# Visual-Behavior/detr-tensorflow

Measured on AMD Instinct MI355X. Metric: images/sec training step, DETR-R50 800x1333 bs=8/GPU, higher is better.
Workload: dtype bf16

## Files before the change

detr-tensorflow_amd/detr_tf/_hip.py:

```python
import ctypes
import os
from ctypes import POINTER, Structure, byref, c_float, c_int32, c_int64, c_size_t, c_void_p

import torch

_HERE = os.path.dirname(os.path.abspath(__file__))
LIB_PATH = os.environ.get("DETR_HIP_LIB") or os.path.join(os.path.dirname(_HERE), "lib", "libdetr_hip.so")

f32p = c_void_p


class ReduceDesc(Structure):
    _fields_ = [("ws", c_void_p), ("splits", c_int32), ("part_stride", c_int64), ("rows", c_int32), ("cols", c_int32),
                ("C", c_void_p), ("ldc", c_int64), ("alpha", c_float), ("scale", c_void_p),
                ("rs_ws", c_void_p), ("rs_out", c_void_p), ("rs_alpha", c_float),
                ("ts_bm", c_int32), ("ts_bn", c_int32), ("ts_tiles_n", c_int32)]


class GemmDesc(Structure):
    _fields_ = [("M", c_int32), ("N", c_int32), ("K", c_int32),
                ("A", c_void_p), ("lda", c_int64), ("a_kcontig", c_int32),
                ("B", c_void_p), ("ldb", c_int64), ("b_kcontig", c_int32),
                ("C", c_void_p), ("ldc", c_int64),
                ("batch", c_int32), ("batch_inner", c_int32),
# ... 179 lines not shown

class SetLossDesc(Structure):
    _fields_ = [("levels", c_int32), ("B", c_int32), ("Q", c_int32), ("C", c_int32), ("R", c_int32),
                ("logits", c_void_p), ("sL_l", c_int64), ("sL_b", c_int64), ("sL_q", c_int64),
                ("boxes", c_void_p), ("sB_l", c_int64), ("sB_b", c_int64), ("sB_q", c_int64),
                ("t_bbox", c_void_p), ("t_class", c_void_p),
                ("background_class", c_int32)]


_SIGNATURES = {
    "detr_hip_abi_version": [],
    "detr_hip_reload_tuning": [],
    "detr_hip_struct_layout": [c_int32, POINTER(c_int32), c_int32],
    "detr_hip_memset_zero": [c_void_p, c_size_t, c_void_p],
    "detr_hip_gemm_f32": [POINTER(GemmDesc), c_void_p],
    "detr_hip_gemm_group_f32": [POINTER(GemmDesc), c_int32, c_void_p],
    "detr_hip_gemm_family": [POINTER(GemmDesc)],
    "detr_hip_gemm_ring_plan": [c_int32, c_int32, c_int32, POINTER(c_int32)],
    "detr_hip_splitk_reduce_many": [POINTER(ReduceDesc), c_int32, c_void_p],
    "detr_hip_conv3x3_f32": [POINTER(Conv3x3Desc), c_int32, c_void_p],
    "detr_hip_maxpool3x3s2_fwd_bf16": [c_void_p, c_void_p, c_void_p, c_int32, c_int32, c_int32, c_int32, c_int32, c_int32, c_void_p],
    "detr_hip_maxpool3x3s2_bwd_bf16": [c_void_p, c_void_p, c_void_p, c_void_p, c_int32, c_int32, c_int32, c_int32, c_int32, c_int32,
                                       c_void_p],
    "detr_hip_cvt_bf16": [f32p, c_void_p, c_int64, c_void_p],
    "detr_hip_scale_cols_bf16": [f32p, f32p, c_void_p, c_int64, c_int32, c_void_p],
    "detr_hip_scale_cols_bf16_group": [c_void_p, c_int32, c_void_p],
    "detr_hip_stem_conv7x7_f32": [POINTER(StemDesc), c_int32, c_void_p],
    "detr_hip_maxpool3x3s2_fwd_f32": [f32p, f32p, c_void_p, c_int32, c_int32, c_int32, c_int32, c_int32, c_int32, c_void_p],
    "detr_hip_maxpool3x3s2_bwd_f32": [f32p, c_void_p, f32p, f32p, c_int32, c_int32, c_int32, c_int32, c_int32, c_int32, c_void_p],
    "detr_hip_subsample2_fwd_f32": [f32p, f32p, c_int32, c_int32, c_int32, c_int32, c_int32, c_int32, c_void_p],
    "detr_hip_subsample2_bwd_f32": [f32p, f32p, c_int32, c_int32, c_int32, c_int32, c_int32, c_int32, c_void_p],
    "detr_hip_layernorm_fwd": [POINTER(LayerNormDesc), c_void_p],
    "detr_hip_layernorm_bwd": [POINTER(LayerNormDesc), c_void_p],
    "detr_hip_attention_fwd": [POINTER(AttnDesc), c_void_p],
    "detr_hip_attention_bwd": [POINTER(AttnDesc), c_void_p],
    "detr_hip_attention_dropmask": [POINTER(AttnDesc), c_void_p],
    "detr_hip_attention_dropmask_many": [POINTER(AttnDesc), c_int32, c_void_p],
    "detr_hip_attention_fwd_masked": [POINTER(AttnDesc), c_void_p, c_void_p],
    "detr_hip_attention_bwd_masked": [POINTER(AttnDesc), c_void_p, c_void_p],
    "detr_hip_attention_weights": [POINTER(AttnDesc), c_void_p, c_void_p, c_int64, c_void_p],
    "detr_hip_padding_mask_prepare": [c_void_p, c_int32, c_int32, c_int32, c_int32, c_int32, f32p, f32p, c_void_p, f32p, c_void_p, c_void_p],
    "detr_hip_input_stage_padded": [c_void_p, c_void_p, c_void_p, c_int32, c_int32, c_int32, f32p, c_void_p, f32p, c_void_p, c_void_p],
    "detr_hip_dropout_f32": [f32p, f32p, c_int64, c_float, ctypes.c_uint32, c_void_p, c_void_p],
    "detr_hip_multi_copy": [c_void_p, c_int32, c_int32, c_void_p],
    "detr_hip_colsum_scaled": [c_void_p, c_int32, c_int64, c_int32, c_int64, c_void_p, c_void_p, c_void_p],
    "detr_hip_fma_vec_group": [c_void_p, c_int32, c_void_p],
    "detr_hip_set_u32x8": [c_void_p] + [ctypes.c_uint32] * 8 + [c_void_p],
    "detr_hip_colsum_f32": [f32p, f32p, c_int64, c_int32, c_int64, c_float, c_void_p],
    "detr_hip_colsum_det_f32": [f32p, f32p, c_int64, c_int32, c_int64, c_float, f32p, c_int64, c_void_p],
    "detr_hip_conv1x1_bwd_fused_bf16": [c_void_p, c_int64, c_void_p, c_int64, c_void_p, c_int64, c_void_p, c_int64, c_int32, f32p, c_int64, f32p, c_float,
                                        c_int64, c_int32, c_int32, f32p, c_int64, c_void_p],
    "detr_hip_add_bcast_f32": [f32p, f32p, f32p, c_int64, c_int64, c_void_p],
    "detr_hip_add_f32": [f32p, f32p, f32p, c_int64, c_void_p],
    "detr_hip_sigmoid_bwd_f32": [f32p, f32p, f32p, c_int64, c_void_p],
    "detr_hip_relu_mask_f32": [f32p, f32p, f32p, c_int64, c_void_p],
    "detr_hip_scale_cols_f32": [f32p, f32p, f32p, c_int64, c_int32, c_void_p],
    "detr_hip_scale_cols_t_f32": [f32p, f32p, f32p, c_int32, c_int32, c_void_p],
    "detr_hip_bn_fold_f32": [f32p, f32p, f32p, f32p, f32p, f32p, c_int32, c_float, c_void_p],
    "detr_hip_postprocess": [POINTER(PostprocessDesc), c_void_p],
    "detr_hip_map_match": [POINTER(MapMatchDesc), c_void_p],
    "detr_hip_input_stage": [POINTER(InputDesc), c_void_p],
    "detr_hip_pad_labels": [c_void_p, c_void_p, c_void_p, c_int32, c_int32, c_void_p, c_void_p, c_void_p],
    "detr_hip_augment": [c_void_p, c_int64, c_void_p, f32p, c_int32, c_int32, c_int32, f32p, c_void_p, f32p, c_void_p],
    "detr_hip_augment_padded": [c_void_p, c_int64, c_void_p, c_int32, c_int32, c_int32, f32p, c_void_p, f32p, c_void_p, c_void_p],
    "detr_hip_match_cost_f32": [POINTER(SetLossDesc), f32p, c_void_p],
    "detr_hip_assign_f32": [f32p, c_int32, c_int32, c_int32, f32p, c_int32, c_int32, c_void_p, c_void_p, c_void_p, c_void_p],
    "detr_hip_set_loss_sums_f32": [POINTER(SetLossDesc), c_void_p, f32p, c_void_p],
    "detr_hip_set_loss_finalize_f32": [f32p, c_int32, f32p, f32p, c_void_p],
    "detr_hip_set_loss_grad_f32": [POINTER(SetLossDesc), c_void_p, f32p, c_float, f32p, f32p, c_void_p],
    "detr_hip_sumsq_segments_f32": [f32p, c_void_p, c_void_p, c_void_p, c_int32, c_int32, f32p, c_void_p],
    "detr_hip_clip_adam_f32": [f32p, f32p, f32p, f32p, c_void_p, c_void_p, c_void_p, c_void_p, f32p, f32p, c_int32, c_int32, c_void_p],
    "detr_hip_axpy_f32": [f32p, f32p, c_float, c_int64, c_void_p],
    "detr_hip_set_floats8_f32": [f32p] + [c_float] * 8 + [c_void_p],
    "detr_hip_set_floats16_f32": [f32p, POINTER(c_float * 16), c_void_p],
    "detr_hip_global_clip_scale_f32": [f32p, c_void_p, c_void_p, f32p, c_int32, f32p, c_void_p],
    "detr_hip_adamw_f32": [f32p, f32p, f32p, f32p, c_void_p, c_void_p, c_void_p, c_void_p, f32p, f32p, f32p, c_int32, c_int32, c_void_p],
    "detr_hip_conv3x3_dilated": [POINTER(Conv3x3DDesc), c_int32, c_void_p],
    "detr_hip_detect": [POINTER(DetectDesc), c_void_p],
    "detr_hip_tile_merge": [POINTER(TileMergeDesc), c_void_p],
    "detr_hip_coco_match": [POINTER(CocoMatchDesc), c_void_p],
    "detr_hip_overlay": [POINTER(OverlayDesc), c_void_p],
    "detr_hip_track": [POINTER(TrackDesc), c_void_p],
    "detr_hip_track_embed": [POINTER(TrackEmbedDesc), c_void_p],
}
_SIGNATURES_I64 = {
    "detr_hip_attention_dropmask_words": [c_int32, c_int32, c_int32, c_int32],
    "detr_hip_attention_keymask_words": [c_int32, c_int32],
    "detr_hip_colsum_det_scratch_floats": [c_int64, c_int32],
    "detr_hip_conv1x1_bwd_fused_workspace_floats": [c_int64],
    "detr_hip_workspace_bytes_gemm": [POINTER(GemmDesc)],
    "detr_hip_workspace_bytes_conv3x3": [POINTER(Conv3x3Desc), c_int32],
    "detr_hip_workspace_bytes_stem": [POINTER(StemDesc), c_int32],
    "detr_hip_workspace_bytes_layernorm": [POINTER(LayerNormDesc)],
    "detr_hip_workspace_bytes_conv3x3_dilated": [POINTER(Conv3x3DDesc), c_int32],
    "detr_hip_workspace_bytes_overlay": [POINTER(OverlayDesc)],
    "detr_hip_track_state_bytes": [c_int32],
    "detr_hip_track_embed_state_bytes": [c_int32, c_int32],
    "detr_hip_workspace_bytes_track_embed": [POINTER(TrackEmbedDesc)],
}
EXPORTED_SYMBOLS = sorted(list(_SIGNATURES) + list(_SIGNATURES_I64) + ["detr_hip_last_error"])
ABI_VERSION = 9
LAYOUT_STRUCTS = {0: ReduceDesc, 1: GemmDesc, 2: Conv3x3Desc, 3: StemDesc, 4: LayerNormDesc, 5: AttnDesc, 6: SetLossDesc, 7: InputDesc,
                  8: PostprocessDesc, 9: MapMatchDesc, 100: DetectDesc, 200: TileMergeDesc, 300: OverlayDesc}
LAYOUT_STRUCTS_APPENDED = {400: TrackDesc}
LAYOUT_STRUCTS_APPENDED_500 = {500: TrackEmbedDesc}

_lib = None


class KernelProfiler:

    def __init__(self, prealloc=0, f32=False):
        self.f32 = f32
        self.records = []
        self._pool = []
        for _ in range(prealloc):
            ev = torch.cuda.Event(enable_timing=True)
            ev.record()
            self._pool.append(ev)

    def _event(self):
        return self._pool.pop() if self._pool else torch.cuda.Event(enable_timing=True)

    def begin(self):
        ev = self._event()
        ev.record()
        return ev

    def end(self, family, flops, ev0, sig=None, nbytes=0.0):
        ev1 = self._event()
        ev1.record()
        self.records.append((family, flops, ev0, ev1, sig, nbytes))

    def by_shape(self, top=40):
        torch.cuda.synchronize()
        agg = {}
        for fam, flops, e0, e1, sig, _nb in self.records:
            d = agg.setdefault((fam, sig), [0, 0.0, 0.0])
            d[0] += 1
            d[1] += e0.elapsed_time(e1)
            d[2] += flops
        rows = sorted(agg.items(), key=lambda kv: -kv[1][1])[:top]
        return [{"family": k[0], "shape": k[1], "launches": v[0], "ms": round(v[1], 3),
                 "tflops": round(v[2] / (v[1] * 1e-3) / 1e12, 2) if v[1] > 0 else 0.0} for k, v in rows]

    def summary(self):
        torch.cuda.synchronize()
        out = {}
        for fam, flops, e0, e1, _sig, nb in self.records:
            d = out.setdefault(fam, {"launches": 0, "ms": 0.0, "flops": 0.0, "bytes": 0.0, "mixed_s": 0.0})
            d["launches"] += 1
            d["ms"] += e0.elapsed_time(e1)
            d["flops"] += flops
            d["bytes"] += nb
            d["mixed_s"] += max(flops / (157.3e12 if fam.startswith("gemm_f32") or self.f32 else 2.5e15), nb / 8.0e12)
        return out


PROFILER = None
DEFER = None
DEFER_WS = None
_defer_top = 0
_defer_outs = set()
COMPUTE_BF16 = 0
WORKSPACE = None

# ... 290 lines not shown
    if COMPUTE_BF16 == 1 and ((N >= 128 and K >= 16384) or (M >= 512 and N >= 512 and K >= 4096) or
                         (K >= 4096 and ((M >= 256 and N >= 2048) or (M >= 2048 and N >= 256)))):
        tiles = -(-M // 128) * -(-N // 128)
        ktiles = -(-K // 32)
        return int(max(1, min(max(1, SPLIT_TARGET_128 // tiles), max_split, ktiles // 8 if ktiles >= 16 else 1)))
    if COMPUTE_BF16 == 2 and X3_SPLIT_TARGET > 0 and N >= 128 and K >= 256 and M >= 128:
        t128 = -(-M // 128) * -(-N // 128)
        ktiles = -(-K // 32)
        cap = ktiles // 8 if ktiles >= 64 else max(1, ktiles // 4)
        s128 = int(max(1, min(X3_SPLIT_TARGET // t128, max_split, cap)))
        if t128 * s128 >= 192:
            return s128
    tiles = -(-M // 64) * -(-N // 64)
    want = max(1, SPLIT_TARGET_64 // max(tiles, 1))
    ktiles = -(-K // (32 if COMPUTE_BF16 == 1 else 16))
    cap = ktiles // 8 if ktiles >= 64 else ktiles // 4
    return int(max(1, min(want, max_split, cap)))


def linear_fwd_call(x2d, w_out_in, bias, out2d, *, alpha=1.0, residual=None, act=0, dropout_p=0.0, dropout_seed=0,
                    dropout_step=None, ln=None):
    M, K = x2d.shape
    N = w_out_in.shape[0]
    return ((M, N, K, x2d, x2d.stride(0), 1, w_out_in, w_out_in.stride(0), 1, out2d, out2d.stride(0)),
            dict(alpha=alpha, bias=bias, residual=residual, ldr=(residual.stride(0) if residual is not None else 0), act=act,
                 dropout_p=dropout_p, dropout_seed=dropout_seed, dropout_step=dropout_step, **({"ln": ln} if ln is not None else {})))


def linear_dgrad_call(dy2d, w_out_in, dx2d, *, alpha=1.0, residual=None, mask=None):
    M, N = dy2d.shape
    K = w_out_in.shape[1]
    return ((M, K, N, dy2d, dy2d.stride(0), 1, w_out_in, w_out_in.stride(0), 0, dx2d, dx2d.stride(0)),
            dict(alpha=alpha, residual=residual, ldr=(residual.stride(0) if residual is not None else 0),
                 mask=mask, ldmask=(mask.stride(0) if mask is not None else 0)))


def linear_wgrad_call(dy2d, x2d, dw_out_in, *, alpha=1.0, bias_grad=None):
    M, N = dy2d.shape
    K = x2d.shape[1]
    sk = pick_split_k(N, K, M)
    args = (N, K, M, dy2d, dy2d.stride(0), 0, x2d, x2d.stride(0), 0, dw_out_in, dw_out_in.stride(0))
    if sk == 1:
        return args, dict(alpha=alpha, residual=dw_out_in, ldr=dw_out_in.stride(0), rowsum_a=bias_grad, rowsum_alpha=alpha)
    return args, dict(alpha=alpha, split_k=sk, rowsum_a=bias_grad, rowsum_alpha=alpha)


def linear_fwd(*a, **kw):
    args, kwargs = linear_fwd_call(*a, **kw)
    gemm(*args, **kwargs)


def linear_dgrad(*a, **kw):
    args, kwargs = linear_dgrad_call(*a, **kw)
    gemm(*args, **kwargs)


def linear_wgrad(*a, **kw):
    args, kwargs = linear_wgrad_call(*a, **kw)
    gemm(*args, **kwargs)


def conv1x1_bwd_fused_scratch_floats(M):
    return int(load().detr_hip_conv1x1_bwd_fused_workspace_floats(int(M)))


def conv1x1_bwd_fused(dy, a, w, da, dw, scratch, *, scale=None, use_mask=True, alpha=1.0):
    M = dy.shape[0]
    for t, shape, dt in ((dy, (M, 256), torch.bfloat16), (a, (M, 64), torch.bfloat16), (w, (64, 256), torch.bfloat16), (da, (M, 64), torch.bfloat16),
                         (dw, (64, 256), torch.float32)):
        if tuple(t.shape) != shape or t.dtype != dt or t.stride(1) != 1:
            raise ValueError(f"conv1x1_bwd_fused: operand of shape {tuple(t.shape)} / {t.dtype} / strides {t.stride()}, expected {shape} {dt}, unit column stride")
    if scratch.dtype != torch.float32 or (scale is not None and (scale.dtype != torch.float32 or scale.numel() != 256)):
        raise ValueError("conv1x1_bwd_fused: scratch / scale must be fp32 (scale: 256 entries)")
    ev0 = PROFILER.begin() if PROFILER is not None else None
    _check(load().detr_hip_conv1x1_bwd_fused_bf16(dy.data_ptr(), dy.stride(0), a.data_ptr(), a.stride(0), w.data_ptr(), w.stride(0), da.data_ptr(),
                                                  da.stride(0), 1 if use_mask else 0, dw.data_ptr(), dw.stride(0), ptr(scale), c_float(alpha), M,
                                                  a.shape[1], dy.shape[1], scratch.data_ptr(), scratch.numel(), _stream()),
           "detr_hip_conv1x1_bwd_fused_bf16")
    if ev0 is not None:
        PROFILER.end("conv1x1_bwd_fused", 4.0 * M * a.shape[1] * dy.shape[1], ev0, f"M{M} {a.shape[1]}->{dy.shape[1]}",
                     float(2 * M * (dy.shape[1] + 2 * a.shape[1])))


def conv3x3(mode, x, w, y, N, Hi, Wi, Ci, Ho, Wo, Co, stride, *, pad=1, alpha=1.0, scale=None, bias=None,
            residual=None, mask=None, act=0, split=0, compute=None, maskbits_out=None, dilation=1):
    if dilation not in (1, 2):
        raise ValueError(f"conv3x3: dilation {dilation} unsupported (1 or 2)")
    dil = dilation == 2
    d = Conv3x3DDesc() if dil else Conv3x3Desc()
    if dil:
        d.dilation = 2
    fn, ws_fn = ("detr_hip_conv3x3_dilated", "detr_hip_workspace_bytes_conv3x3_dilated") if dil else \
        ("detr_hip_conv3x3_f32", "detr_hip_workspace_bytes_conv3x3")
    d.N, d.Hi, d.Wi, d.Ci, d.Ho, d.Wo, d.Co, d.stride, d.pad = N, Hi, Wi, Ci, Ho, Wo, Co, stride, pad
    d.x, d.w, d.y = x.data_ptr(), w.data_ptr(), y.data_ptr()
    is16 = lambda t: 1 if (t is not None and t.dtype == torch.bfloat16) else 0
    d.w_dtype, d.x_dtype, d.y_dtype, d.r_dtype, d.m_dtype = is16(w), is16(x), is16(y), is16(residual), is16(mask)
    if mask is not None and mask.dtype == torch.uint8:
        d.m_dtype = 2
    d.maskbits_out = ptr(maskbits_out)
    d.alpha = alpha
    d.scale, d.bias, d.residual, d.mask = ptr(scale), ptr(bias), ptr(residual), ptr(mask)
    d.act, d.split = act, split
    d.compute = COMPUTE_BF16 if compute is None else int(compute)
    if mode == 2 and WORKSPACE is not None:
        need_workspace(_ws_query(ws_fn, ("convd" if dil else "conv", N, Hi, Wi, Ci, Ho, Wo, Co, stride, pad, split, d.compute, d.x_dtype),
                                 byref(d), mode))
    d.workspace, d.workspace_bytes = (WORKSPACE.data_ptr(), WORKSPACE.numel() * 4) if WORKSPACE is not None else (None, 0)
    ev0 = PROFILER.begin() if PROFILER is not None else None
    _check(getattr(load(), fn)(byref(d), mode, _stream()), fn)
    if ev0 is not None:
        rows = N * (Hi * Wi if mode == 1 else Ho * Wo)
        PROFILER.end(("conv3x3_fwd", "conv3x3_dgrad", "conv3x3_wgrad")[mode], 2.0 * (N * Ho * Wo) * 9 * Ci * Co, ev0,
                     f"N{N} {Hi}x{Wi}x{Ci}->{Ho}x{Wo}x{Co} s{stride}" + (" d2" if dil else ""),
                     float(x.element_size() * (N * Hi * Wi * Ci if mode != 1 else N * Ho * Wo * Co)
                           + (w.element_size() * 9 * Ci * Co if mode != 2 else w.element_size() * N * Ho * Wo * Co)
                           + y.element_size() * (N * Ho * Wo * Co if mode == 0 else (N * Hi * Wi * Ci if mode == 1 else 9 * Ci * Co))
                           + ((rows * (Ci if mode == 1 else Co) // 8 if mask.dtype == torch.uint8 else mask.element_size() * rows * (Ci if mode == 1 else Co))
                              if mask is not None else 0) + (rows * Co // 8 if maskbits_out is not None else 0)
                           + (residual.element_size() * rows * (Ci if mode == 1 else Co) if residual is not None else 0)))


def stem_conv(mode, img, w, y, N, H, W, Ho, Wo, *, alpha=1.0, scale=None, bias=None, act=0, split=0, compute=None):
    d = StemDesc()
    d.N, d.H, d.W, d.Ho, d.Wo = N, H, W, Ho, Wo
    d.img, d.w, d.y = img.data_ptr(), w.data_ptr(), y.data_ptr()
    d.alpha = alpha
    d.scale, d.bias = ptr(scale), ptr(bias)
    d.act, d.split = act, split
    d.w_dtype = 1 if (mode == 2 and w.dtype == torch.bfloat16) else 0
    d.y_dtype = 1 if (mode == 0 and y.dtype == torch.bfloat16) else 0
    d.compute = COMPUTE_BF16 if compute is None else int(compute)
    if mode == 2 and WORKSPACE is not None:
        need_workspace(_ws_query("detr_hip_workspace_bytes_stem", ("stem", N, H, W, Ho, Wo, split, d.compute, d.w_dtype), byref(d), mode))
    d.workspace, d.workspace_bytes = (WORKSPACE.data_ptr(), WORKSPACE.numel() * 4) if WORKSPACE is not None else (None, 0)
    ev0 = PROFILER.begin() if PROFILER is not None else None
    _check(load().detr_hip_stem_conv7x7_f32(byref(d), mode, _stream()), "detr_hip_stem_conv7x7_f32")
    if ev0 is not None:
        M = N * Ho * Wo
        PROFILER.end("stem_conv7x7", 2.0 * M * 64 * 147, ev0, f"stem7x7 mode{mode} M{M}",
                     float(4 * N * H * W * 3 + (y if mode == 0 else w).element_size() * M * 64 + 4 * 147 * 64))


def call(name, *args):
    _check(getattr(load(), name)(*args, _stream()), name)


def zero_(t):
    call("detr_hip_memset_zero", t.data_ptr(), t.numel() * t.element_size())
    return t


def attention_dropmask_words(B, H, T, S):
    return int(load().detr_hip_attention_dropmask_words(B, H, T, S))


def attention_keymask_words(B, S):
    return int(load().detr_hip_attention_keymask_words(B, S))


def keymask_words_from_valid(valid):
    import numpy as np
    valid = np.asarray(valid, dtype=bool)
    B, S = valid.shape
    nw = (S + 31) // 32
    bits = np.zeros((B, nw * 32), dtype=np.uint64)
# ... 180 lines not shown
```

detr-tensorflow_amd/detr_tf/engine.py:

```python
import math
import os
from ctypes import byref, c_float

import numpy as np
import torch

from . import _hip as hip
from .params import ParamStore, RESNET50_BLOCKS, block_names, bn_conv_pairs, stem_names

D = 256
HEADS = 8
HD = 32
FF = 2048
BN_EPS = 1e-5
KERAS_BN_EPS = 1.001e-5
LN_EPS = 1e-5
DEFER_REDUCE = os.environ.get("DETR_HIP_DEFER_REDUCE", "1") != "0"
WGRAD_STREAM = os.environ.get("DETR_HIP_WGRAD_STREAM", "1") != "0"
BWD_FUSED = os.environ.get("DETR_HIP_BWD_FUSED", "1") != "0"
DROPMASK_AHEAD = int(os.environ.get("DETR_HIP_DROPMASK_AHEAD", "2") or 0)
QK_ALPHA = float(HD) ** -0.5 * 1.4426950408889634


def mix32(x):
    x &= 0xFFFFFFFF
    x ^= x >> 16
    x = (x * 0x7FEB352D) & 0xFFFFFFFF
    x ^= x >> 15
    x = (x * 0x846CA68B) & 0xFFFFFFFF
    x ^= x >> 16
    return x


def step_seed(base_seed, step_no, rank=0):
    return mix32(mix32((base_seed + 0x9E3779B9 * step_no) & 0xFFFFFFFF) ^ ((rank * 0x85EBCA6B) & 0xFFFFFFFF))


def position_embedding_sine_host(H, W, num_pos_features=128, temperature=10000.0, eps=1e-6):
    y = (np.arange(1, H + 1, dtype=np.float32) / np.float32(H + eps) * np.float32(2 * math.pi)).astype(np.float32)
    x = (np.arange(1, W + 1, dtype=np.float32) / np.float32(W + eps) * np.float32(2 * math.pi)).astype(np.float32)
    k = np.arange(num_pos_features, dtype=np.float32)
    dim_t = np.power(np.float32(temperature), (2 * np.floor(k / 2) / np.float32(num_pos_features)).astype(np.float32)).astype(np.float32)
    py = (y[:, None] / dim_t[None, :]).astype(np.float32)
    px = (x[:, None] / dim_t[None, :]).astype(np.float32)
    ey = np.empty_like(py)
    ex = np.empty_like(px)
    ey[:, 0::2], ey[:, 1::2] = np.sin(py[:, 0::2]), np.cos(py[:, 1::2])
    ex[:, 0::2], ex[:, 1::2] = np.sin(px[:, 0::2]), np.cos(px[:, 1::2])
    pos = np.concatenate([np.broadcast_to(ey[:, None, :], (H, W, num_pos_features)),
                          np.broadcast_to(ex[None, :, :], (H, W, num_pos_features))], axis=2)
    return np.ascontiguousarray(pos.reshape(H * W, 2 * num_pos_features), dtype=np.float32)


def position_embedding_sine_table(n_max, num_pos_features=128, temperature=10000.0, eps=1e-6):
    k = np.arange(num_pos_features, dtype=np.float32)
    dim_t = np.power(np.float32(temperature), (2 * np.floor(k / 2) / np.float32(num_pos_features)).astype(np.float32)).astype(np.float32)
    tab = np.zeros((n_max + 1, n_max + 1, num_pos_features), np.float32)
    c = np.arange(0, n_max + 1, dtype=np.float32)
    for n in range(n_max + 1):
        y = (c / np.float32(n + eps) * np.float32(2 * math.pi)).astype(np.float32)
        py = (y[:, None] / dim_t[None, :]).astype(np.float32)
        tab[n, :, 0::2], tab[n, :, 1::2] = np.sin(py[:, 0::2]), np.cos(py[:, 1::2])
    return tab


def downsample_mask_nearest(mask, Hf, Wf):
    mask = np.asarray(mask)
    H, W = mask.shape[1:]
    sy = np.minimum((np.arange(Hf) * H) // Hf, H - 1)
    sx = np.minimum((np.arange(Wf) * W) // Wf, W - 1)
    return mask[:, sy][:, :, sx]


def dilation_flags(replace_stride_with_dilation):
    if replace_stride_with_dilation is None:
        return (False, False, False)
    flags = tuple(bool(f) for f in replace_stride_with_dilation)
    if len(flags) != 3:
        raise ValueError(f"replace_stride_with_dilation: expected 3 flags (layer2, layer3, layer4), got {len(flags)}")
    return flags


def feature_size(H, W, replace_stride_with_dilation=None):
    for halves in (True, True) + tuple(not f for f in dilation_flags(replace_stride_with_dilation)):
        if halves:
            H, W = (H - 1) // 2 + 1, (W - 1) // 2 + 1
    return H, W


def backbone_stride(replace_stride_with_dilation=None):
    return 4 * 2 ** sum(1 for f in dilation_flags(replace_stride_with_dilation) if not f)


class DetrEngine:
    def __init__(self, device="cuda:0", blocks=RESNET50_BLOCKS, num_enc=6, num_dec=6, num_queries=100,
                 num_classes=92, nb_class=None, seed=0, tf_backbone=False, replace_stride_with_dilation=(False, False, False)):
        self.dilate = dilation_flags(replace_stride_with_dilation)
        if tf_backbone and any(self.dilate):
            raise ValueError("replace_stride_with_dilation needs the reference backbone: tf.keras.applications.ResNet50 "
                             "(tf_backbone=True) has no such option")
        hip.load()
        self.device = torch.device(device)
# ... 450 lines not shown
                    hip.flush_reduces()
                    on_bucket(i)
        elif on_bucket:
            def cb(i):
                self._side_join()
                on_bucket(i)
        self._side_begin(WGRAD_STREAM and DEFER_REDUCE and d_logits.is_cuda)
        try:
            return self._backward_impl(d_logits, d_boxes, backbone, cb)
        finally:
            try:
                self._side_join()
                self._side_on = False
                hip.flush_reduces(end=True)
            finally:
                hip.COMPUTE_BF16 = 0

    def _prepare_masks(self, masks, B, H, W, Hf, Wf):
        L = Hf * Wf
        if tuple(masks.shape) != (B, H, W) or masks.dtype not in (torch.uint8, torch.bool):
            raise ValueError(f"masks: expected a uint8 / bool tensor of shape {(B, H, W)}, got {masks.dtype} {tuple(masks.shape)}")
        key = (Hf, Wf)
        if key not in self._pos_tables:
            self._pos_tables[key] = (torch.from_numpy(position_embedding_sine_table(Hf)).to(self.device),
                                     torch.from_numpy(position_embedding_sine_table(Wf)).to(self.device))
        tab_y, tab_x = self._pos_tables[key]
        kv = self.buf("mask:key_valid", (B * ((L + 31) // 32),), torch.int32)
        pos = self.buf("mask:pos", (B * L, D))
        status = self.buf("mask:status", (B,), torch.int32)
        hip.padding_mask_prepare(masks, Hf, Wf, tab_y, tab_x, kv, pos, status)
        self.key_valid = kv
        return pos

    def _host_masks(self, masks, shape):
        host = np.asarray(masks.cpu() if torch.is_tensor(masks) else masks).astype(bool)
        if host.shape != shape:
            raise ValueError(f"masks: expected shape {shape}, got {host.shape}")
        Hf, Wf = feature_size(shape[1], shape[2], self.dilate)
        empty = [b for b in range(shape[0]) if downsample_mask_nearest(host[b:b + 1], Hf, Wf).all()]
        if empty:
            raise ValueError(f"masks: image(s) {empty} have no valid (unpadded) position on the {Hf} x {Wf} feature map")
        return torch.from_numpy(host.view(np.uint8)).to(self.device)

    def check_mask_status(self):
        if self.key_valid is None:
            return
        st = self._bufs["mask:status"].cpu()
        bad = [int(b) for b in torch.nonzero(st).flatten()]
        if bad:
            raise ValueError(f"masks: image(s) {bad} have no valid (unpadded) position on the feature map")

    def _forward_impl(self, images, training=False, masks=None):
        assert images.is_cuda and images.dtype == torch.float32 and images.dim() == 4 and images.shape[3] == 3
        images = images.contiguous()
        if training and self.dropout_p > 0.0:
            if not self._graph_replay:
                self.advance_dropout_step()
            self._drop = (float(self.dropout_p), self._step_seed)
        else:
            self._drop = (0.0, 0)
        dp, dseed = self._drop
        B, H, W, _ = images.shape
        self._shape = (B, H, W)
        if dp > 0.0:
            hf, wf = feature_size(H, W, self.dilate)
            self._gen_dropmasks(B, hf * wf)
        self.images = images
        V = self.P.views
        self.phase("fwd backbone")
        H1, W1 = (H + 6 - 7) // 2 + 1, (W + 6 - 7) // 2 + 1
        M1 = B * H1 * W1
        ws = self._scaled_kernel(f"{self._stem['conv']}/kernel", self._stem["bn"])
        adt = torch.bfloat16 if self.compute == 1 else torch.float32
        self._adt = adt
        stem = self.buf("stem:out", (B, H1, W1, 64), adt)
        hip.stem_conv(0, images, ws, stem, B, H, W, H1, W1, bias=self.bn_shift[self._stem["bn"]], act=1)
        H2, W2 = (H1 + 2 - 3) // 2 + 1, (W1 + 2 - 3) // 2 + 1
        pool = self.buf("stem:pool", (B, H2, W2, 64), adt)
        amax = self.buf("stem:amax", (B, H2, W2, 64), torch.uint8)
        hip.call("detr_hip_maxpool3x3s2_fwd_bf16" if adt == torch.bfloat16 else "detr_hip_maxpool3x3s2_fwd_f32", stem.data_ptr(),
                 pool.data_ptr(), amax.data_ptr(), B, H1, W1, 64, H2, W2)
        x, h, w, cin = pool, H2, W2, 64
        self._block_meta = []
        for li, nb in enumerate(self.blocks):
            d1, d2 = 64 * 2 ** li, 256 * 2 ** li
            for b in range(nb):
                n = block_names(li, b, self.tf_backbone)
                p = n["tag"]
                dilated = li > 0 and self.dilate[li - 1]
                stride = 2 if (b == 0 and li > 0 and not dilated) else 1
                dil = 2 if (dilated and b > 0) else 1
                ho, wo = (h - 1) // stride + 1, (w - 1) // stride + 1
                M_in, M_out = B * h * w, B * ho * wo
                xs = x
                if stride == 2 and (b == 0):
                    xs = self.buf(f"{p}:xs", (B, ho, wo, cin), adt)
                    hip.call("detr_hip_subsample2_fwd_f32", x.data_ptr(), xs.data_ptr(), B, h, w,
                             cin // 2 if adt == torch.bfloat16 else cin, ho, wo)
                if self.tf_backbone:
                    x1, M1, h1, w1, s2 = xs, M_out, ho, wo, 1
                else:
                    x1, M1, h1, w1, s2 = x, M_in, h, w, stride
                if b == 0:
                    idn = self.buf(f"{p}:idn", (B, ho, wo, d2), adt)
                    self._side(lambda: self._conv1x1_fwd(xs, M_out, cin, d2, f"{n['down']}/kernel", n["bnd"], idn, act=0))
                else:
                    idn = x
                y1 = self.buf(f"{p}:y1", (B, h1, w1, d1), adt)
                self._conv1x1_fwd(x1, M1, cin, d1, f"{n['conv1']}/kernel", n["bn1"], y1)
                y2 = self.buf(f"{p}:y2", (B, ho, wo, d1), adt)
                hip.conv3x3(0, y1, self._scaled_kernel(f"{n['conv2']}/kernel", n["bn2"]), y2, B, h1, w1, d1, ho, wo, d1,
                            s2, bias=self.bn_shift[n["bn2"]], act=1, pad=dil, dilation=dil)
                if b == 0:
                    self._side_join()
                out = self.buf(f"{p}:out", (B, ho, wo, d2), adt)
                nxt_d1 = 64 * 2 ** (li if b + 1 < nb else li + 1)
                last = (li + 1 == len(self.blocks)) and (b + 1 == nb)
                obits = self.buf(f"{p}:out_bits", (M_out, d2 // 8), torch.uint8) \
                    if (training and adt == torch.bfloat16 and not last and nxt_d1 <= 256) else None
                self._conv1x1_fwd(y2, M_out, d1, d2, f"{n['conv3']}/kernel", n["bn3"], out, residual=idn, maskbits_out=obits)
                self._block_meta.append(dict(p=p, n=n, x=x, xs=xs, x1=x1, y1=y1, y2=y2, out=out, h=h, w=w, ho=ho, wo=wo, h1=h1, w1=w1,
                                             M1=M1, s2=s2, cin=cin, d1=d1, d2=d2, stride=stride, first=(b == 0), out_bits=obits, dil=dil))
                x, h, w, cin = out, ho, wo, d2
        feat, Hf, Wf = x, h, w
        L = Hf * Wf
        self._feat_meta = (feat, Hf, Wf, L)
        self.phase("fwd encoder")
        src = self.buf("enc:src0", (B * L, D))
        hip.gemm(B * L, D, 2048, feat, 2048, 1, self._w("input_proj/kernel"), D, 0, src, D, bias=V["input_proj/bias"])
        key = (Hf, Wf)
        if masks is None:
            self.key_valid = None
            if key not in self._pos_cache:
                self._pos_cache[key] = torch.from_numpy(position_embedding_sine_host(Hf, Wf)).to(self.device)
            pos = self._pos_cache[key]
        else:
            pos = self._prepare_masks(masks, B, H, W, Hf, Wf)
        self.pos = pos
        x = src
        qk = self.buf("enc0:qk", (B * L, D))
        self._add_bcast(x, pos, qk)
        for i in range(self.num_enc):
            pfx, tag = f"transformer/encoder/layer_{i}", f"enc{i}"
            a = self.buf(f"{tag}:a", (B * L, D))
            x1 = self.buf(f"{tag}:x1", (B * L, D))
            x1h = self.buf(f"{tag}:x1h", (B * L, D), torch.bfloat16) if self.ffn16 else None
            ln1 = self._ln_spec(B * L, f"{pfx}/norm1", x1, f"{tag}:ln1", y16=x1h)
            self._self_attn_fwd(f"{tag}:sa", f"{pfx}/self_attn", qk, x, B, L, a, site=16 * i, ln=ln1, key_valid=self.key_valid)
            if ln1 is None:
                self._ln_fwd(a, f"{pfx}/norm1", x1, f"{tag}:ln1", y16=x1h)
            f = self.buf(f"{tag}:f", (B * L, D))
            x2 = self.buf(f"{tag}:x2", (B * L, D))
            qk = self.buf(f"enc{i + 1}:qk" if i + 1 < self.num_enc else "dec:mem_pos", (B * L, D))
            ln2 = self._ln_spec(B * L, f"{pfx}/norm2", x2, f"{tag}:ln2", add=pos, y2=qk, ffn=True)
            self._ffn_fwd(tag, pfx, x1, f, seed=16 * i + 2, x16=x1h, ln=ln2)
            if ln2 is None:
                self._ln_fwd(f, f"{pfx}/norm2", x2, f"{tag}:ln2", add=pos, y2=qk)
            x = x2
        memory, mem_pos = x, qk
        if self.num_enc == 0:
            mem_pos = qk
        self.phase("fwd decoder")
        if training:
            self._pregen_dropmasks(B, L)
        Q, nd = self.Q, self.num_dec
        qpos = V["query_embed/kernel"]
        tgt = self.buf("dec:tgt0", (B * Q, D))
        hip.zero_(tgt)
        hs = self.buf("dec:hs", (nd, B * Q, D))
        t3all = self.buf("dec:t3all", (nd, B * Q, D))
        dp, _ = self._drop
        ct = self._cross_tables()
        if self._stale(f"cross:{self.compute}"):
            hip.multi_copy(ct["gather"])
        a16 = self.attn16
        KV = self.buf("dec:KV16" if a16 else "dec:KV", (B * L, 2 * nd * D), torch.bfloat16 if a16 else torch.float32)
        self._side(lambda: hip.gemm_group([hip.linear_fwd_call(mem_pos, ct["Wkv"][0:nd * D], ct["bkv"][0:nd * D], KV[:, 0:nd * D]),
                                           hip.linear_fwd_call(memory, ct["Wkv"][nd * D:], ct["bkv"][nd * D:], KV[:, nd * D:])]))
        qin = self.buf("dec0:qin", (B * Q, D))
        self._add_bcast(tgt, qpos, qin)
        for i in range(nd):
            pfx, tag = f"transformer/decoder/layer_{i}", f"dec{i}"
            ds = 16 * (32 + i)
            a1 = self.buf(f"{tag}:a1", (B * Q, D))
            t1 = self.buf(f"{tag}:t1", (B * Q, D))
            q2 = self.buf(f"{tag}:q2", (B * Q, D))
            ln1 = self._ln_spec(B * Q, f"{pfx}/norm1", t1, f"{tag}:ln1", add=qpos, y2=q2)
            self._self_attn_fwd(f"{tag}:sa", f"{pfx}/self_attn", qin, tgt, B, Q, a1, site=ds, ln=ln1)
            if ln1 is None:
                self._ln_fwd(a1, f"{pfx}/norm1", t1, f"{tag}:ln1", add=qpos, y2=q2)
            cp = f"{pfx}/multihead_attn"
            Wc, bc = self._w(f"{cp}/in_proj_kernel"), V[f"{cp}/in_proj_bias"]
            Qc = self.buf(f"{tag}:ca:Q16" if a16 else f"{tag}:ca:Q", (B * Q, D), torch.bfloat16 if a16 else torch.float32)
            hip.linear_fwd(q2, Wc[0:D], bc[0:D], Qc, alpha=QK_ALPHA if a16 else 1.0)
            if i == 0:
                self._side_join()
            Oc = self.buf(f"{tag}:ca:O16" if a16 else f"{tag}:ca:O", (B * Q, D), torch.bfloat16 if a16 else torch.float32)
            lse = self.buf(f"{tag}:ca:lse", (B * HEADS, Q))
            hip.attention(Qc, KV[:, i * D:(i + 1) * D], KV[:, (nd + i) * D:(nd + i + 1) * D], Oc, lse, B, HEADS, Q, L,
                          scale=float(HD) ** -0.5, dropout_p=dp, dropout_site=ds + 2, dropout_step=self._seed_dev,
                          dropmask=self._dropmask(ds + 2, B, Q, L) if (a16 and dp > 0.0) else None, key_valid=self.key_valid)
            if cp in self._attn_sites:
                self._attn_map(cp, Qc, KV[:, i * D:(i + 1) * D], lse, B, Q, L, self.key_valid)
# ... 317 lines not shown
```

include/detr_hip.h:

```cpp
#ifndef DETR_HIP_H
#define DETR_HIP_H

#include <stddef.h>
#include <stdint.h>

#ifdef __cplusplus
extern "C" {
#endif

#define DETR_HIP_ABI_VERSION 9

const char *detr_hip_last_error(void);
int detr_hip_abi_version(void);
int detr_hip_reload_tuning(void);
int detr_hip_struct_layout(int32_t which, int32_t *out, int32_t cap);
int detr_hip_memset_zero(void *ptr, size_t bytes, void *stream);

typedef struct detr_reduce_desc {
    const float *ws; int32_t splits; int64_t part_stride; int32_t rows, cols;
    float *C; int64_t ldc; float alpha; const float *scale;
    const float *rs_ws; float *rs_out; float rs_alpha;
    int32_t ts_bm, ts_bn, ts_tiles_n;
} detr_reduce_desc;

// ... 408 lines not shown
    int32_t glyph_digit0, glyph_colon, glyph_dot;
    const int32_t *scale;
    const float *heat;
    int64_t sH_b, sH_y, sH_x;
    int32_t Hf, Wf;
    const float *map_step;
    const int32_t *map_valid;
    const float *map_scale;
    const uint8_t *lut;
    int32_t heat_alpha;
    void *workspace;
    int64_t workspace_bytes;
    int32_t *status;
} detr_overlay_desc;
int detr_hip_overlay(const detr_overlay_desc *d, void *stream);
int64_t detr_hip_workspace_bytes_overlay(const detr_overlay_desc *d);

#define DETR_TRACK_MAX 256
#define DETR_TRACK_FULL 1
#define DETR_TRACK_BAD_COUNT 2
typedef struct {
    int32_t S, D;
    void *state;
    int64_t state_bytes;
    const float *boxes;
    const int64_t *labels;
    const float *scores;
    const int32_t *query;
    const int32_t *counts;
    const int32_t *active;
    float track_threshold, new_threshold;
    double match_threshold, low_match_threshold;
    int32_t max_age, min_hits;
    float alpha, beta;
    int32_t class_agnostic;
    float *out_boxes;
    int64_t *out_labels;
    float *out_scores;
    int32_t *out_query, *out_ids, *out_hits;
    int32_t *out_counts;
    int32_t *status;
} detr_track_desc;
int detr_hip_track(const detr_track_desc *d, void *stream);
int64_t detr_hip_track_state_bytes(int32_t streams);

#define DETR_TRACK_BAD_EMBED 4
typedef struct {
    int32_t S, D;
    void *state;
    int64_t state_bytes;
    const float *boxes;
    const int64_t *labels;
    const float *scores;
    const int32_t *query;
    const int32_t *counts;
    const int32_t *active;
    float track_threshold, new_threshold;
    double match_threshold, low_match_threshold;
    int32_t max_age, min_hits;
    float alpha, beta;
    int32_t class_agnostic;
    float *out_boxes;
    int64_t *out_labels;
    float *out_scores;
    int32_t *out_query, *out_ids, *out_hits;
    int32_t *out_counts;
    int32_t *status;
    const float *embed;
    int64_t sE_s, sE_r;
    int32_t R, E;
    void *embed_state;
    int64_t embed_state_bytes;
    void *workspace;
    int64_t workspace_bytes;
    double appearance_weight;
    int32_t reid;
    double reid_threshold;
    float momentum;
} detr_track_embed_desc;
int detr_hip_track_embed(const detr_track_embed_desc *d, void *stream);
int64_t detr_hip_track_embed_state_bytes(int32_t streams, int32_t embed_dim);
int64_t detr_hip_workspace_bytes_track_embed(const detr_track_embed_desc *d);

#ifdef __cplusplus
}
#endif
#endif
```

Measured before the change: 530.2.

## Fuse bottleneck conv3 with next block's conv1 in a paired streaming GEMM

Adds a persistent HIP kernel that computes a block's conv3 1x1 GEMM (64->256, with bias, residual add, ReLU, and optional mask bits) and feeds the bf16 result straight into the next block's conv1 (256->64, bias, ReLU) from LDS. The engine uses it in layer1 blocks where both shapes match, then skips the separate conv1 launch in the following block. This removes one kernel launch and one full re-read of the 256-channel activation from global memory per fused pair. The cost is a more complex kernel held to one workgroup per CU by its large LDS footprint, plus extra ABI surface.

```diff
diff --git a/detr-tensorflow_amd/csrc/gemm_pair.h b/detr-tensorflow_amd/csrc/gemm_pair.h
--- /dev/null
+++ b/detr-tensorflow_amd/csrc/gemm_pair.h
@@ -0,0 +1,214 @@
+#pragma once
+#include "gemm_stream.h"
+
+namespace detr {
+
+struct PairArgs {
+    int M;
+    const unsigned short *A; long long lda;
+    const unsigned short *B1; long long ldb1;
+    const unsigned short *B2; long long ldb2;
+    unsigned short *Y; long long ldy;
+    unsigned short *Z; long long ldz;
+    const unsigned short *res; long long ldr;
+    unsigned char *mbits; long long ld_mbits;
+    const float *bias1, *bias2;
+    int row_tiles;
+    int stride;
+};
+
+constexpr int PAIR_K1 = 64, PAIR_N1 = 256, PAIR_WAVES = 8, PAIR_M_MIN = 16384;
+
+template <int N2>
+struct PairSmem {
+    unsigned short B1[PAIR_N1 / 64][64][PAIR_K1 + 8];
+    unsigned short B2[N2 / 64][64][PAIR_N1 + 8];
+    float bias1[PAIR_N1];
+    float stage[PAIR_WAVES][32][STREAM_LD];
+};
+
+template <int N2, bool MBO>
+__global__ __launch_bounds__(64 * PAIR_WAVES, 1) void gemm_pair_bf16_kernel(PairArgs a) {
+    constexpr int THREADS = 64 * PAIR_WAVES, KK = 4, NS = PAIR_N1 / 64, NQ2 = N2 / 32;
+    static_assert(N2 == 64, "gemm_pair: the second epilogue is written for one 64-column slice");
+    static_assert(sizeof(PairSmem<N2>) <= 160 * 1024, "gemm_pair: LDS");
+    __shared__ __attribute__((aligned(16))) PairSmem<N2> sm;
+    const int tid = threadIdx.x, lane = tid & 63, wave = tid >> 6;
+    const int l31 = lane & 31, h = lane >> 5;
+    const int erow = lane >> 3, ecg = lane & 7;
+    const int stride = a.stride;
+
+    BufSrc srcA, srcR, dstY, dstZ, dstB;
+    srcA.init_bytes(a.A, ((long long)(a.M - 1) * a.lda + PAIR_K1) * 2);
+    srcR.init_bytes(a.res, ((long long)(a.M - 1) * a.ldr + PAIR_N1) * 2);
+    dstY.init_bytes(a.Y, ((long long)(a.M - 1) * a.ldy + PAIR_N1) * 2);
+    dstZ.init_bytes(a.Z, ((long long)(a.M - 1) * a.ldz + N2) * 2);
+    if (MBO) dstB.init_bytes(a.mbits, (long long)(a.M - 1) * a.ld_mbits + PAIR_N1 / 8);
+    const unsigned ldy2 = (unsigned)(a.ldy * 2), ldz2 = (unsigned)(a.ldz * 2), ldr2 = (unsigned)(a.ldr * 2), ldb1 = (unsigned)a.ld_mbits;
+    float bias2[8];
+#pragma unroll
+    for (int i = 0; i < 8; ++i) bias2[i] = a.bias2 ? a.bias2[ecg * 8 + i] : 0.0f;
+    float *stage = &sm.stage[wave][0][0];
+    const unsigned a_lane = (unsigned)(h * 16);
+
+    auto load_a = [&](int rt, uint4 (&f)[KK]) {
+        const int row = rt * 32 + l31;
+        const unsigned base = (rt < a.row_tiles && row < a.M) ? (unsigned)((long long)row * a.lda * 2) + a_lane : BUF_OOB;
+#pragma unroll
+        for (int kk = 0; kk < KK; ++kk) f[kk] = srcA.ld16(base == BUF_OOB ? BUF_OOB : base + kk * 32);
+    };
+    auto load_res = [&](int rt, int s, uint4 (&r)[4]) {
+#pragma unroll
+        for (int it = 0; it < 4; ++it) {
+            const int row = rt * 32 + it * 8 + erow;
+            r[it] = stream_ld_ep(srcR, (rt < a.row_tiles && row < a.M) ? (unsigned)row * ldr2 + (unsigned)((s * 64 + ecg * 8) * 2) : BUF_OOB);
+        }
+    };
+    auto mma4 = [&](auto nq_tag, const unsigned short *img, int img_elems, int ks0, const uint4 (&f)[KK], auto &acc) {
+        constexpr int NQ = decltype(nq_tag)::value;
+        auto read_b = [&](int kk, int nq) -> bf16x8 {
+            return frag_tr<64>(reinterpret_cast<const unsigned short(*)[8]>(img + (nq >> 1) * img_elems), (nq & 1) * 32, ks0 + kk * 16, lane);
+        };
+        bf16x8 bq[2][NQ];
+#pragma unroll
+        for (int nq = 0; nq < NQ; ++nq) bq[0][nq] = read_b(0, nq);
+        sgb_ds_read<2 * NQ>();
+#pragma unroll
+        for (int kk = 0; kk < KK; ++kk) {
+            const bf16x8 af = __builtin_bit_cast(bf16x8, f[kk]);
+#pragma unroll
+            for (int nq = 0; nq < NQ; ++nq) {
+                if (kk + 1 < KK) bq[(kk + 1) & 1][nq] = read_b(kk + 1, nq);
+                acc[nq] = __builtin_amdgcn_mfma_f32_32x32x16_bf16(bq[kk & 1][nq], af, acc[nq], 0, 0, 0);
+            }
+#pragma unroll
+            for (int nq = 0; nq < NQ; ++nq) {
+                if (kk + 1 < KK) sgb_ds_read<2>();
+                sgb_mfma();
+            }
+        }
+    };
+    auto transpose = [&](const f32x16 (&acc)[2]) {
+#pragma unroll
+        for (int nh = 0; nh < 2; ++nh)
+#pragma unroll
+            for (int g = 0; g < 4; ++g)
+                *reinterpret_cast<float4 *>(stage + l31 * STREAM_LD + nh * 32 + 8 * g + 4 * h) =
+                    make_float4(acc[nh][4 * g], acc[nh][4 * g + 1], acc[nh][4 * g + 2], acc[nh][4 * g + 3]);
+        __builtin_amdgcn_fence(__ATOMIC_SEQ_CST, "wavefront");
+        __builtin_amdgcn_wave_barrier();
+    };
+
+    auto strip = [&](const int rt, uint4 (&a_cur)[KK], uint4 (&rres)[2][4]) {
+        const int r0 = rt * 32;
+        f32x16 acc2[NQ2];
+#pragma unroll
+        for (int nq = 0; nq < NQ2; ++nq)
+#pragma unroll
+            for (int r = 0; r < 16; ++r) acc2[nq][r] = 0.0f;
+#pragma unroll
+        for (int s = 0; s < NS; ++s) {
+            if (s + 1 < NS) load_res(rt, s + 1, rres[(s + 1) & 1]);
+            else load_res(rt + stride, 0, rres[0]);
+            f32x16 acc[2];
+#pragma unroll
+            for (int nq = 0; nq < 2; ++nq)
+#pragma unroll
+                for (int r = 0; r < 16; ++r) acc[nq][r] = 0.0f;
+            mma4(std::integral_constant<int, 2>{}, &sm.B1[s][0][0], 0, 0, a_cur, acc);
+            if (s + 1 == NS) load_a(rt + stride, a_cur);
+            transpose(acc);
+            const float4 b0 = *reinterpret_cast<const float4 *>(&sm.bias1[s * 64 + ecg * 8]);
+            const float4 b1 = *reinterpret_cast<const float4 *>(&sm.bias1[s * 64 + ecg * 8 + 4]);
+            const float bias[8] = {b0.x, b0.y, b0.z, b0.w, b1.x, b1.y, b1.z, b1.w};
+#pragma unroll
+            for (int it = 0; it < 4; ++it) {
+                const int rl = it * 8 + erow;
+                const int row = r0 + rl;
+                const float4 v0 = *reinterpret_cast<const float4 *>(stage + rl * STREAM_LD + ecg * 8);
+                const float4 v1 = *reinterpret_cast<const float4 *>(stage + rl * STREAM_LD + ecg * 8 + 4);
+                float v[8] = {v0.x, v0.y, v0.z, v0.w, v1.x, v1.y, v1.z, v1.w};
+                float r[8];
+                stream_unpack8(rres[s & 1][it], r);
+#pragma unroll
+                for (int i = 0; i < 8; ++i) v[i] = vmax_raw((v[i] + bias[i]) + r[i], 0.0f);
+                const bool st_live = row < a.M;
+                const u32x4 ov = {f32_to_bf16_pair(v[0], v[1]), f32_to_bf16_pair(v[2], v[3]), f32_to_bf16_pair(v[4], v[5]), f32_to_bf16_pair(v[6], v[7])};
+                dstY.st16(st_live ? (unsigned)row * ldy2 + (unsigned)((s * 64 + ecg * 8) * 2) : BUF_OOB, ov);
+                if constexpr (MBO)
+                    dstB.st1(st_live ? (unsigned)row * ldb1 + (unsigned)(s * 8 + ecg) : BUF_OOB, (unsigned char)bf16x8_gt0_bits(ov[0], ov[1], ov[2], ov[3]));
+                *reinterpret_cast<u32x4 *>(reinterpret_cast<unsigned short *>(stage + rl * STREAM_LD) + ecg * 8) = ov;
+            }
+            __builtin_amdgcn_fence(__ATOMIC_SEQ_CST, "wavefront");
+            __builtin_amdgcn_wave_barrier();
+            uint4 yf[KK];
+#pragma unroll
+            for (int kk = 0; kk < KK; ++kk)
+                yf[kk] = *reinterpret_cast<const uint4 *>(reinterpret_cast<const unsigned short *>(stage + l31 * STREAM_LD) + kk * 16 + h * 8);
+            __builtin_amdgcn_fence(__ATOMIC_SEQ_CST, "wavefront");
+            __builtin_amdgcn_wave_barrier();
+            mma4(std::integral_constant<int, NQ2>{}, &sm.B2[0][0][0], 64 * (PAIR_N1 + 8), s * 64, yf, acc2);
+        }
+        transpose(acc2);
+#pragma unroll
+        for (int it = 0; it < 4; ++it) {
+            const int rl = it * 8 + erow;
+            const int row = r0 + rl;
+            const float4 v0 = *reinterpret_cast<const float4 *>(stage + rl * STREAM_LD + ecg * 8);
+            const float4 v1 = *reinterpret_cast<const float4 *>(stage + rl * STREAM_LD + ecg * 8 + 4);
+            float v[8] = {v0.x, v0.y, v0.z, v0.w, v1.x, v1.y, v1.z, v1.w};
+#pragma unroll
+            for (int i = 0; i < 8; ++i) v[i] = vmax_raw(v[i] + bias2[i], 0.0f);
+            const u32x4 ov = {f32_to_bf16_pair(v[0], v[1]), f32_to_bf16_pair(v[2], v[3]), f32_to_bf16_pair(v[4], v[5]), f32_to_bf16_pair(v[6], v[7])};
+            dstZ.st16(row < a.M ? (unsigned)row * ldz2 + (unsigned)(ecg * 16) : BUF_OOB, ov);
+        }
+        __builtin_amdgcn_fence(__ATOMIC_SEQ_CST, "wavefront");
+        __builtin_amdgcn_wave_barrier();
+    };
+
+    int rt = blockIdx.x * PAIR_WAVES + wave;
+    uint4 a0[KK], rres[2][4];
+    load_a(rt, a0);
+    load_res(rt, 0, rres[0]);
+
+    for (int c = tid; c < PAIR_K1 * (PAIR_N1 / 8); c += THREADS) {
+        const int k = c / (PAIR_N1 / 8), nc = c - k * (PAIR_N1 / 8);
+        const uint4 v = *reinterpret_cast<const uint4 *>(a.B1 + (long long)k * a.ldb1 + nc * 8);
+        const int ncl = nc & 7;
+        unsigned short *img = &sm.B1[nc >> 3][0][0];
+        *reinterpret_cast<uint4 *>(img + (((k >> 2) * 4 + (ncl >> 1)) * 64 + (k & 3) * 16 + (ncl & 1) * 8)) = v;
+    }
+    for (int c = tid; c < PAIR_N1 * (N2 / 8); c += THREADS) {
+        const int k = c / (N2 / 8), nc = c - k * (N2 / 8);
+        const uint4 v = *reinterpret_cast<const uint4 *>(a.B2 + (long long)k * a.ldb2 + nc * 8);
+        const int ncl = nc & 7;
+        unsigned short *img = &sm.B2[nc >> 3][0][0];
+        *reinterpret_cast<uint4 *>(img + (((k >> 2) * 4 + (ncl >> 1)) * 64 + (k & 3) * 16 + (ncl & 1) * 8)) = v;
+    }
+    for (int c = tid; c < PAIR_N1; c += THREADS) sm.bias1[c] = a.bias1 ? a.bias1[c] : 0.0f;
+    __syncthreads();
+
+    while (rt < a.row_tiles) {
+        strip(rt, a0, rres);
+        rt += stride;
+    }
+}
+
+static inline int gemm_pair_workgroups(long long M) {
+    const long long row_tiles = (M + 31) / 32;
+    long long wgs = row_tiles / (PAIR_WAVES * 2);
+    if (wgs > 256) wgs = 256;
+    if (wgs < 1) wgs = 1;
+    return (int)wgs;
+}
+
+template <int N2>
+static void launch_gemm_pair(PairArgs a, hipStream_t s) {
+    const int wgs = gemm_pair_workgroups(a.M);
+    a.row_tiles = (a.M + 31) / 32;
+    a.stride = wgs * PAIR_WAVES;
+    if (a.mbits) hipLaunchKernelGGL((gemm_pair_bf16_kernel<N2, true>), dim3((unsigned)wgs), dim3(64 * PAIR_WAVES), 0, s, a);
+    else hipLaunchKernelGGL((gemm_pair_bf16_kernel<N2, false>), dim3((unsigned)wgs), dim3(64 * PAIR_WAVES), 0, s, a);
+}
+
+}
diff --git a/detr-tensorflow_amd/csrc/gemm_pair.hip b/detr-tensorflow_amd/csrc/gemm_pair.hip
--- /dev/null
+++ b/detr-tensorflow_amd/csrc/gemm_pair.hip
@@ -0,0 +1,42 @@
+#include <type_traits>
+#include "common.h"
+#include "gemm_pair.h"
+
+using namespace detr;
+
+extern "C" int detr_hip_gemm_pair_fwd_stride(int64_t M) {
+    if (M < PAIR_M_MIN || M >= (1ll << 31)) return -1;
+    return gemm_pair_workgroups(M) * PAIR_WAVES;
+}
+
+extern "C" int detr_hip_gemm_pair_fwd_bf16(const uint16_t *a, int64_t lda, const uint16_t *w1, int64_t ldw1, const float *bias1, const uint16_t *res,
+                                           int64_t ldr, uint16_t *y, int64_t ldy, uint8_t *ybits, int64_t ld_ybits, const uint16_t *w2, int64_t ldw2,
+                                           const float *bias2, uint16_t *z, int64_t ldz, int64_t M, int32_t K1, int32_t N1, int32_t N2,
+                                           int32_t act_dtype, int32_t w_dtype, int64_t col_stride, void *stream) {
+    DETR_REQUIRE(a && w1 && res && y && w2 && z, "gemm pair: a, w1, res, y, w2 and z are required");
+    DETR_REQUIRE(K1 == PAIR_K1 && N1 == PAIR_N1 && N2 == 64, "gemm pair: built for %d -> %d -> 64 channels, got %d -> %d -> %d", PAIR_K1, PAIR_N1, K1, N1, N2);
+    DETR_REQUIRE(act_dtype == 1 && w_dtype == 1 && col_stride == 1, "gemm pair: bf16 operands with contiguous columns only (dtypes %d / %d, column stride %lld)",
+                 act_dtype, w_dtype, (long long)col_stride);
+    DETR_REQUIRE(M >= PAIR_M_MIN && M < (1ll << 31), "gemm pair: M = %lld is outside the streaming range (at least %d rows)", (long long)M, PAIR_M_MIN);
+    DETR_REQUIRE(lda >= K1 && ldw1 >= N1 && ldr >= N1 && ldy >= N1 && ldw2 >= N2 && ldz >= N2 && (!ybits || ld_ybits >= N1 / 8) && lda % 8 == 0 &&
+                 ldw1 % 8 == 0 && ldr % 8 == 0 && ldy % 8 == 0 && ldw2 % 8 == 0 && ldz % 8 == 0, "gemm pair: leading dimensions");
+    DETR_REQUIRE(aligned16(a) && aligned16(w1) && aligned16(res) && aligned16(y) && aligned16(w2) && aligned16(z), "gemm pair: alignment");
+    long long pitch = lda;
+    for (long long p : {(long long)ldr, (long long)ldy, (long long)ldz, (long long)(ybits ? (ld_ybits + 1) / 2 : 0)})
+        if (p > pitch) pitch = p;
+    DETR_REQUIRE(((M - 1) * pitch + N1) * 2 <= BUF_MAX_BYTES, "gemm pair: operand larger than a buffer descriptor's range (4 GB)");
+    PairArgs k;
+    k.M = (int)M;
+    k.A = a; k.lda = lda;
+    k.B1 = w1; k.ldb1 = ldw1;
+    k.B2 = w2; k.ldb2 = ldw2;
+    k.Y = y; k.ldy = ldy;
+    k.Z = z; k.ldz = ldz;
+    k.res = res; k.ldr = ldr;
+    k.mbits = ybits; k.ld_mbits = ld_ybits;
+    k.bias1 = bias1; k.bias2 = bias2;
+    k.row_tiles = k.stride = 0;
+    launch_gemm_pair<64>(k, (hipStream_t)stream);
+    DETR_LAUNCH_CHECK("gemm pair");
+    return 0;
+}
diff --git a/detr-tensorflow_amd/detr_tf/_hip.py b/detr-tensorflow_amd/detr_tf/_hip.py
--- a/detr-tensorflow_amd/detr_tf/_hip.py
+++ b/detr-tensorflow_amd/detr_tf/_hip.py
@@ -285,6 +285,9 @@
     "detr_hip_overlay": [POINTER(OverlayDesc), c_void_p],
     "detr_hip_track": [POINTER(TrackDesc), c_void_p],
     "detr_hip_track_embed": [POINTER(TrackEmbedDesc), c_void_p],
+    "detr_hip_gemm_pair_fwd_bf16": [c_void_p, c_int64, c_void_p, c_int64, f32p, c_void_p, c_int64, c_void_p, c_int64, c_void_p, c_int64, c_void_p, c_int64,
+                                    f32p, c_void_p, c_int64, c_int64, c_int32, c_int32, c_int32, c_int32, c_int32, c_int64, c_void_p],
+    "detr_hip_gemm_pair_fwd_stride": [c_int64],
 }
 _SIGNATURES_I64 = {
     "detr_hip_attention_dropmask_words": [c_int32, c_int32, c_int32, c_int32],
@@ -741,6 +744,32 @@
                      float(2 * M * (dy.shape[1] + 2 * a.shape[1])))
 
 
+GEMM_PAIR_MIN_ROWS = 16384
+
+
+def gemm_pair_fwd_stride(M):
+    return int(load().detr_hip_gemm_pair_fwd_stride(int(M)))
+
+
+def gemm_pair_fwd(a, w1, bias1, res, y, w2, bias2, z, *, maskbits_out=None):
+    M, K1 = a.shape
+    N1, N2 = w1.shape[1], w2.shape[1]
+    acts, wts = (a, res, y, z), (w1, w2)
+    act_dtype = 1 if all(t.dtype == torch.bfloat16 for t in acts) else 0
+    w_dtype = 1 if all(t.dtype == torch.bfloat16 for t in wts) else 0
+    col_stride = max(t.stride(1) for t in acts + wts)
+    ev0 = PROFILER.begin() if PROFILER is not None else None
+    _check(load().detr_hip_gemm_pair_fwd_bf16(a.data_ptr(), a.stride(0), w1.data_ptr(), w1.stride(0), ptr(bias1), res.data_ptr(), res.stride(0),
+                                              y.data_ptr(), y.stride(0), ptr(maskbits_out), maskbits_out.stride(0) if maskbits_out is not None else 0,
+                                              w2.data_ptr(), w2.stride(0), ptr(bias2), z.data_ptr(), z.stride(0), M, K1, N1, N2, act_dtype, w_dtype,
+                                              col_stride, _stream()),
+           "detr_hip_gemm_pair_fwd_bf16")
+    if ev0 is not None:
+        nbytes = 2.0 * (M * K1 + K1 * N1 + N1 * N2 + 2 * M * N1 + M * N2) + (M * N1 // 8 if maskbits_out is not None else 0)
+        PROFILER.end("gemm_stream_bf16_kernel", 2.0 * M * (K1 * N1 + N1 * N2), ev0,
+                     f"pair M{M} N{N1} K{K1} -> N{N2} res{' bits' if maskbits_out is not None else ''}", nbytes)
+
+
 def conv3x3(mode, x, w, y, N, Hi, Wi, Ci, Ho, Wo, Co, stride, *, pad=1, alpha=1.0, scale=None, bias=None,
             residual=None, mask=None, act=0, split=0, compute=None, maskbits_out=None, dilation=1):
     if dilation not in (1, 2):
diff --git a/detr-tensorflow_amd/detr_tf/engine.py b/detr-tensorflow_amd/detr_tf/engine.py
--- a/detr-tensorflow_amd/detr_tf/engine.py
+++ b/detr-tensorflow_amd/detr_tf/engine.py
@@ -18,6 +18,7 @@
 DEFER_REDUCE = os.environ.get("DETR_HIP_DEFER_REDUCE", "1") != "0"
 WGRAD_STREAM = os.environ.get("DETR_HIP_WGRAD_STREAM", "1") != "0"
 BWD_FUSED = os.environ.get("DETR_HIP_BWD_FUSED", "1") != "0"
+PAIR_FWD = os.environ.get("DETR_HIP_PAIR_FWD", "1") != "0"
 DROPMASK_AHEAD = int(os.environ.get("DETR_HIP_DROPMASK_AHEAD", "2") or 0)
 QK_ALPHA = float(HD) ** -0.5 * 1.4426950408889634
 
@@ -634,6 +635,7 @@
                  pool.data_ptr(), amax.data_ptr(), B, H1, W1, 64, H2, W2)
         x, h, w, cin = pool, H2, W2, 64
         self._block_meta = []
+        pair_y1 = None
         for li, nb in enumerate(self.blocks):
             d1, d2 = 64 * 2 ** li, 256 * 2 ** li
             for b in range(nb):
@@ -659,7 +661,11 @@
                 else:
                     idn = x
                 y1 = self.buf(f"{p}:y1", (B, h1, w1, d1), adt)
-                self._conv1x1_fwd(x1, M1, cin, d1, f"{n['conv1']}/kernel", n["bn1"], y1)
+                if pair_y1 is None:
+                    self._conv1x1_fwd(x1, M1, cin, d1, f"{n['conv1']}/kernel", n["bn1"], y1)
+                else:
+                    assert pair_y1 is y1 and x1 is x
+                    pair_y1 = None
                 y2 = self.buf(f"{p}:y2", (B, ho, wo, d1), adt)
                 hip.conv3x3(0, y1, self._scaled_kernel(f"{n['conv2']}/kernel", n["bn2"]), y2, B, h1, w1, d1, ho, wo, d1,
                             s2, bias=self.bn_shift[n["bn2"]], act=1, pad=dil, dilation=dil)
@@ -670,7 +676,15 @@
                 last = (li + 1 == len(self.blocks)) and (b + 1 == nb)
                 obits = self.buf(f"{p}:out_bits", (M_out, d2 // 8), torch.uint8) \
                     if (training and adt == torch.bfloat16 and not last and nxt_d1 <= 256) else None
-                self._conv1x1_fwd(y2, M_out, d1, d2, f"{n['conv3']}/kernel", n["bn3"], out, residual=idn, maskbits_out=obits)
+                if (PAIR_FWD and self.compute == 1 and adt == torch.bfloat16 and not self.tf_backbone and not last and d1 == 64 and d2 == 256
+                        and nxt_d1 == 64 and M_out >= hip.GEMM_PAIR_MIN_ROWS):
+                    nn = block_names(li, b + 1, self.tf_backbone)
+                    pair_y1 = self.buf(f"{nn['tag']}:y1", (B, ho, wo, nxt_d1), adt)
+                    hip.gemm_pair_fwd(y2.view(M_out, d1), self._scaled_kernel(f"{n['conv3']}/kernel", n["bn3"]).view(d1, d2), self.bn_shift[n["bn3"]],
+                                      idn.view(M_out, d2), out.view(M_out, d2), self._scaled_kernel(f"{nn['conv1']}/kernel", nn["bn1"]).view(d2, nxt_d1),
+                                      self.bn_shift[nn["bn1"]], pair_y1.view(M_out, nxt_d1), maskbits_out=obits)
+                else:
+                    self._conv1x1_fwd(y2, M_out, d1, d2, f"{n['conv3']}/kernel", n["bn3"], out, residual=idn, maskbits_out=obits)
                 self._block_meta.append(dict(p=p, n=n, x=x, xs=xs, x1=x1, y1=y1, y2=y2, out=out, h=h, w=w, ho=ho, wo=wo, h1=h1, w1=w1,
                                              M1=M1, s2=s2, cin=cin, d1=d1, d2=d2, stride=stride, first=(b == 0), out_bits=obits, dil=dil))
                 x, h, w, cin = out, ho, wo, d2
diff --git a/include/detr_hip.h b/include/detr_hip.h
--- a/include/detr_hip.h
+++ b/include/detr_hip.h
@@ -514,6 +514,12 @@
 int64_t detr_hip_track_embed_state_bytes(int32_t streams, int32_t embed_dim);
 int64_t detr_hip_workspace_bytes_track_embed(const detr_track_embed_desc *d);
 
+int detr_hip_gemm_pair_fwd_bf16(const uint16_t *a, int64_t lda, const uint16_t *w1, int64_t ldw1, const float *bias1, const uint16_t *res,
+                                int64_t ldr, uint16_t *y, int64_t ldy, uint8_t *ybits, int64_t ld_ybits, const uint16_t *w2, int64_t ldw2,
+                                const float *bias2, uint16_t *z, int64_t ldz, int64_t M, int32_t K1, int32_t N1, int32_t N2,
+                                int32_t act_dtype, int32_t w_dtype, int64_t col_stride, void *stream);
+int detr_hip_gemm_pair_fwd_stride(int64_t M);
+
 #ifdef __cplusplus
 }
 #endif
```

Result: no change. 532.2, median of 6 (+0.4%).
